# dohlee/metheor

Hardware: AMD Instinct MI355X
Metric: M reads/sec (PDR+LPMD, 150bp WGBS) (higher is better)
Workload: dtype u32; 1 GPU; S-chr19-10M (BASELINE config 2): 10000000 x 150bp reads/GPU, chr19 58.6 Mbp, 2.94 CpG calls/read, fused PDR+LPMD, reference CLI defaults; reads_per_gpu=10000000, cpg_calls_per_gpu=29424182, sites_emitted=726028, parallelism=contig-sharded x1

## Files before the change

metheor_amd/csrc/mth_pdr_lpmd.hip:

```cpp
#include "mth_ctx.h"
#include "mth_tile_dev.h"

#ifndef MTH_TILE_PF
#define MTH_TILE_PF 1
#endif

namespace mth {


constexpr int IDX_GROUPS = 1;
__device__ __forceinline__ void index_safe_hi(const uint32_t *__restrict__ cpg_off, const uint32_t n_reads, const uint32_t n_cpgs,
                                              const uint32_t gtid, DevState *__restrict__ st) {
    uint32_t best = 0;
#pragma unroll
    for (uint32_t k = 0; k < 4; ++k) {
        const uint32_t back = gtid * 4u + k;
        if (back <= n_reads) {
            const uint32_t r = n_reads - back;
            if ((uint64_t)cpg_off[r] + 8u <= (uint64_t)n_cpgs) best = max(best, r);
        }
    }
#pragma unroll
    for (int o = 32; o > 0; o >>= 1) best = max(best, (uint32_t)__shfl_xor((int)best, o, 64));
    if (gtid == 0) st->safe_hi = best;
// ... 218 lines not shown
    if (tid < 4) {
        uint32_t s = 0;
        for (int w = 0; w < B / 64; ++w) s += red[tid][w];
        if (s) atomicAdd(a.bucket + a.nbk + (size_t)(t >> TILE_BUCKET_SHIFT) * 4 + tid, (unsigned long long)s);
    }
}

template <int W, int B, bool WIDE>
__device__ __forceinline__ uint32_t tile_compact(const TileArgs &a, const uint32_t t, const int32_t P0, const uint32_t Wp,
                                                 const uint32_t *cnt, uint32_t *wave_off, const uint32_t out_base) {
    const int tid = threadIdx.x, lane = tid & 63, wave = tid >> 6;
    constexpr int NPOS = WIDE ? W / 2 : W;
    constexpr int PER = NPOS / B;
    static_assert(PER % 4 == 0 && PER <= 32, "uint4 LDS reads, 32-bit mask");
    uint32_t qual = 0;
    if (WIDE) {
#pragma unroll
        for (int q = 0; q < PER / 4; ++q) {
            const uint4 x = reinterpret_cast<const uint4 *>(cnt)[tid * (PER / 4) + q];
            const uint4 y = reinterpret_cast<const uint4 *>(cnt + W / 2)[tid * (PER / 4) + q];
            const uint4 cov = make_uint4(x.x + y.x, x.y + y.y, x.z + y.z, x.w + y.w);
            qual |= (cov.x >= a.min_cov ? 1u : 0u) << (4 * q);
            qual |= (cov.y >= a.min_cov ? 1u : 0u) << (4 * q + 1);
            qual |= (cov.z >= a.min_cov ? 1u : 0u) << (4 * q + 2);
            qual |= (cov.w >= a.min_cov ? 1u : 0u) << (4 * q + 3);
        }
    } else {
        uint32_t below = 0;
#ifdef MTH_TILE_ROT
        static_assert(PER == 16 || WIDE, "the rotation is written for 16 positions per thread");
        const uint32_t rot = ((uint32_t)lane >> 2) & 3u;
#pragma unroll
        for (int q = PER / 4 - 1; q >= 0; --q) {
            const uint4 x = reinterpret_cast<const uint4 *>(cnt)[tid * (PER / 4) + (((uint32_t)q + rot) & 3u)];
            below = __builtin_amdgcn_alignbit(below, (x.w & 0xffffu) - a.min_cov, 31);
            below = __builtin_amdgcn_alignbit(below, (x.z & 0xffffu) - a.min_cov, 31);
            below = __builtin_amdgcn_alignbit(below, (x.y & 0xffffu) - a.min_cov, 31);
            below = __builtin_amdgcn_alignbit(below, (x.x & 0xffffu) - a.min_cov, 31);
        }
        {
            const uint32_t dbl = below | (below << 16);
            below = (dbl >> (16u - 4u * rot)) & 0xffffu;
        }
#else
#pragma unroll
        for (int q = PER / 4 - 1; q >= 0; --q) {
            const uint4 x = reinterpret_cast<const uint4 *>(cnt)[tid * (PER / 4) + q];
            below = __builtin_amdgcn_alignbit(below, (x.w & 0xffffu) - a.min_cov, 31);
            below = __builtin_amdgcn_alignbit(below, (x.z & 0xffffu) - a.min_cov, 31);
            below = __builtin_amdgcn_alignbit(below, (x.y & 0xffffu) - a.min_cov, 31);
            below = __builtin_amdgcn_alignbit(below, (x.x & 0xffffu) - a.min_cov, 31);
        }
#endif
        qual = ~below & (PER == 32 ? 0xffffffffu : (1u << PER) - 1u);
    }
    {
        const int32_t left = (int32_t)Wp - tid * PER;
        qual &= left >= PER ? 0xffffffffu : (left > 0 ? (1u << left) - 1u : 0u);
    }
    const uint32_t mine = __builtin_popcount(qual);
    const uint32_t incl = wave_scan_incl(mine);
    static_assert(B == 256, "four wave totals in one 16-byte LDS word");
    if (lane == 63) wave_off[wave] = incl;
    __syncthreads();
    const uint4 wt = *reinterpret_cast<const uint4 *>(wave_off);
    const uint32_t before = (wave > 0 ? wt.x : 0u) + (wave > 1 ? wt.y : 0u) + (wave > 2 ? wt.z : 0u);
    const uint32_t total = wt.x + wt.y + wt.z + wt.w;
    uint32_t o = out_base + before + incl - mine;
    SiteRec *__restrict__ out = a.scratch + (size_t)t * W;
    while (qual) {
        const uint32_t idx = (uint32_t)tid * PER + (uint32_t)__builtin_ctz(qual);
        qual &= qual - 1;
        SiteRec rr; rr.pos = P0 + (int32_t)idx; rr.pad = 0;
        if (WIDE) { rr.n_conc = cnt[idx]; rr.n_disc = cnt[W / 2 + idx]; }
        else { const uint32_t x = cnt[idx]; rr.n_disc = x >> 16; rr.n_conc = (x & 0xffffu) - rr.n_disc; }
        out[o++] = rr;
    }
    return total;
}

template <typename RelT, int NB>
__device__ __forceinline__ void load_rel(const RelT *__restrict__ rp, int32_t (&r)[NB]) {
    if constexpr (sizeof(RelT) == 1) {
#pragma unroll
        for (int k8 = 0; k8 < NB / 8; ++k8) {
            const u32x2_a1 x = *reinterpret_cast<const u32x2_a1 *>(rp + 8 * k8);
#pragma unroll
            for (int k = 0; k < 4; ++k) { r[8 * k8 + k] = (int32_t)((x.x >> (8 * k)) & 0xffu); r[8 * k8 + 4 + k] = (int32_t)((x.y >> (8 * k)) & 0xffu); }
        }
    } else {
#pragma unroll
        for (int k8 = 0; k8 < NB / 8; ++k8) {
            const u32x4_a2 x = *reinterpret_cast<const u32x4_a2 *>(rp + 8 * k8);
            r[8 * k8] = (int32_t)(x.x & 0xffffu); r[8 * k8 + 1] = (int32_t)(x.x >> 16);
            r[8 * k8 + 2] = (int32_t)(x.y & 0xffffu); r[8 * k8 + 3] = (int32_t)(x.y >> 16);
            r[8 * k8 + 4] = (int32_t)(x.z & 0xffffu); r[8 * k8 + 5] = (int32_t)(x.z >> 16);
            r[8 * k8 + 6] = (int32_t)(x.w & 0xffffu); r[8 * k8 + 7] = (int32_t)(x.w >> 16);
        }
    }
}

#ifdef MTH_TILE_TRACE
#define g_tk4 (*mth_tk4p)
#define g_tk5 (*mth_tk5p)
__device__ unsigned long long mth_tk_dummy[2];
#endif
template <int W, int B, int NB, typename RelT, bool WIDE, bool CLAMP, int MG>
__device__ __forceinline__ uint32_t tile_pass(const TileArgs &a, const uint32_t t, const int32_t T0, const int32_t T1,
                                              const int32_t P0, const uint32_t Wp, const uint32_t lo, const uint32_t hi,
                                              const bool do_lp, const uint32_t out_base, uint32_t *cnt_raw,
                                              uint32_t (*red)[B / 64], uint32_t *wave_off, SlotTabs &tabs
#ifdef MTH_TILE_TRACE
                                              , unsigned long long *mth_tk4p = &mth_tk_dummy[0], unsigned long long *mth_tk5p = &mth_tk_dummy[1]
#endif
                                              ) {
    const int tid = threadIdx.x;
    uint32_t *const cnt = cnt_raw + MG;
    constexpr bool MARGIN = MG > 0 && !WIDE;
    const RelT *__restrict__ rel = reinterpret_cast<const RelT *>(a.cpg_rel);
    constexpr bool PACKED = sizeof(RelT) == 1 && NB == 8;

    uint32_t lp_c = 0, lp_d = 0, n_read = 0, n_valid = 0, bad = 0;
    uint32_t i = lo + tid;
    int32_t s = 0;
    uint32_t o0 = 0, n = 0, mq = 0;
    constexpr bool PF = MTH_TILE_PF && !CLAMP && sizeof(RelT) == 1 && NB == 8;
    uint32_t o1 = 0;
    if (PF) { if (i < hi) { o0 = a.cpg_off[i]; o1 = a.cpg_off[i + 1]; } }
    else if (i < hi) { s = a.read_start[i]; o0 = a.cpg_off[i]; n = a.cpg_off[i + 1] - o0; mq = a.read_mapq[i]; }
    while (i < hi) {
        const uint32_t inext = i + B;
        const bool more = inext < hi;
        uint32_t v[NB];
        int32_t r[NB];
        uint32_t rraw0 = 0, rraw1 = 0;
        uint32_t o0n = 0, o1n = 0;
        if constexpr (PF) {
            n = o1 - o0;
            const uint32_t *__restrict__ cp = a.cpg_pos + o0;
#pragma unroll
            for (int k4 = 0; k4 < NB / 4; ++k4) {
                const u32x4_a4 x = *reinterpret_cast<const u32x4_a4 *>(cp + 4 * k4);
                v[4 * k4] = x.x; v[4 * k4 + 1] = x.y; v[4 * k4 + 2] = x.z; v[4 * k4 + 3] = x.w;
            }
            if (do_lp) { const u32x2_a1 x = *reinterpret_cast<const u32x2_a1 *>(reinterpret_cast<const RelT *>(a.cpg_rel) + o0); rraw0 = x.x; rraw1 = x.y; }
            s = a.read_start[i]; mq = a.read_mapq[i];
            if (more) { o0n = a.cpg_off[inext]; o1n = a.cpg_off[inext + 1]; }
        }
        const bool owned = (s >= T0) && (s < T1);
        const bool lp_ok = do_lp && owned && (mq >= a.lpmd_min_qual);
        if (do_lp && owned) { n_read += 1; n_valid += lp_ok ? 1u : 0u; }
        const bool pdr_ok = a.want_pdr && (n >= a.min_cpgs) && (mq >= a.pdr_min_qual) && (n > 0);
        const bool work = (lp_ok || pdr_ok) && n != 0;
        const int32_t maxd = PACKED ? min(a.max_dist, 255) : min(a.max_dist, 1 << 20);
        const int32_t mind = max(a.min_dist, 0);
        const bool any_lp = maxd >= a.min_dist && maxd >= 0 && __any(work && lp_ok && n > 1);
        if (work) {
            const uint32_t *__restrict__ cp = a.cpg_pos + o0;
            const RelT *__restrict__ rp = rel + o0;
            if (PF) {
                (void)cp; (void)rp;
            } else if (!CLAMP) {
#pragma unroll
                for (int k4 = 0; k4 < NB / 4; ++k4) {
                    const u32x4_a4 x = *reinterpret_cast<const u32x4_a4 *>(cp + 4 * k4);
                    v[4 * k4] = x.x; v[4 * k4 + 1] = x.y; v[4 * k4 + 2] = x.z; v[4 * k4 + 3] = x.w;
                }
                if (any_lp) {
                    if constexpr (PACKED) { const u32x2_a1 x = *reinterpret_cast<const u32x2_a1 *>(rp); rraw0 = x.x; rraw1 = x.y; }
                    else load_rel<RelT, NB>(rp, r);
                }
            } else {
#pragma unroll
                for (int k = 0; k < NB; ++k) v[k] = cp[min((uint32_t)k, n - 1)];
                if (any_lp) {
#pragma unroll
                    for (int k = 0; k < NB; ++k) {
                        const uint32_t rv = (uint32_t)rp[min((uint32_t)k, n - 1)];
                        if constexpr (PACKED) { if (k < 4) rraw0 |= rv << (8 * k); else rraw1 |= rv << (8 * (k - 4)); }
                        else r[k] = (int32_t)rv;
                    }
                }
            }
        const uint32_t sm1 = (uint32_t)(s - 1);
        const uint32_t dead_w = ((MARGIN ? (uint32_t)(P0 - MG + (tid & 63)) : (uint32_t)T0 + (1u << 28)) & 0x7fffffffu) | (v[0] & 0x80000000u);
        const uint32_t n_lp = lp_ok ? min(n, (uint32_t)NB) : 0u;
        uint32_t acc = 0, xmax = (v[0] & 0x7fffffffu) - sm1;
        if constexpr (PACKED) {
            const uint32_t nrow = min(n, 8u);
            const uint4 ma = reinterpret_cast<const uint4 *>(&tabs.mtab[nrow][0])[0], mb = reinterpret_cast<const uint4 *>(&tabs.mtab[nrow][0])[1];
            const uint32_t mk[8] = {ma.x, ma.y, ma.z, ma.w, mb.x, mb.y, mb.z, mb.w};
            uint32_t xs[8];
            xs[0] = xmax;
#pragma unroll
            for (int k = 1; k < 8; ++k) {
                xs[k] = __builtin_amdgcn_bitop3_b32(v[k] - sm1, mk[k], 0x7fffffffu, 0x80);
                v[k] = __builtin_amdgcn_bitop3_b32(v[k], dead_w, mk[k], 0xe4);
                acc = __builtin_amdgcn_bitop3_b32(acc, v[k], v[0], 0xf6);
            }
            xmax = max(max(max(xs[0], xs[1]), max(xs[2], xs[3])), max(max(xs[4], xs[5]), max(xs[6], xs[7])));
        } else {
// ... 51 lines not shown
                    const int32_t dist = rk - (int32_t)rel[o0 + j];
                    if (dist > a.max_dist) break;
                    if (dist < a.min_dist) continue;
                    if ((a.cpg_pos[o0 + j] >> 31) == mk) lp_c += 1; else lp_d += 1;
                }
            }
        }
        if (MARGIN) {
            if (pdr_ok && !bad_it && (uint32_t)s - (uint32_t)(P0 - MG + 1) <= (uint32_t)(W + MG - 1)) {
                const uint32_t one = disc ? 0x10001u : 1u;
                const uint32_t base4 = (uint32_t)(P0 - MG) << 2;
#pragma unroll
                for (int k = 0; k < NB; ++k)
                    atomicAdd(reinterpret_cast<uint32_t *>(reinterpret_cast<char *>(cnt_raw) + ((v[k] << 2) - base4)), one);
                if (any_long) {
                    for (uint32_t k = NB; k < n; ++k) {
                        const uint32_t pk = (a.cpg_pos[o0 + k] & 0x7fffffffu) - (uint32_t)P0;
                        if (pk < Wp) atomicAdd(cnt + pk, one);
                    }
                }
            }
        } else if (!WIDE) {
            const uint32_t one = disc ? 0x10001u : 1u;
            const uint32_t base4 = ((uint32_t)P0 << 2) - (pdr_ok ? 0u : (1u << 30));
            const uint32_t trash4 = (uint32_t)(W + (tid & 63)) << 2;
#pragma unroll
            for (int k = 0; k < NB; ++k) {
                const uint32_t a4 = min((v[k] << 2) - base4, trash4);
                atomicAdd(reinterpret_cast<uint32_t *>(reinterpret_cast<char *>(cnt) + a4), one);
            }
            if (any_long && pdr_ok) {
                for (uint32_t k = NB; k < n; ++k) {
                    const uint32_t pk = (a.cpg_pos[o0 + k] & 0x7fffffffu) - (uint32_t)P0;
                    if (pk < Wp) atomicAdd(cnt + pk, one);
                }
            }
        } else {
            const uint32_t wt = pdr_ok ? Wp : 0u;
            const uint32_t dw = disc ? (uint32_t)(W / 2) : 0u;
            const uint32_t trash = (uint32_t)(W + (tid & 63)) - dw;
#pragma unroll
            for (int k = 0; k < NB; ++k) {
                const uint32_t pk = (v[k] & 0x7fffffffu) - (uint32_t)P0;
                atomicAdd(cnt + ((pk < wt ? pk : trash) + dw), 1u);
            }
            if (any_long && pdr_ok) {
                for (uint32_t k = NB; k < n; ++k) {
                    const uint32_t pk = (a.cpg_pos[o0 + k] & 0x7fffffffu) - (uint32_t)P0;
                    if (pk < Wp) atomicAdd(cnt + dw + pk, 1u);
                }
            }
        }
        }
        if (PF) { o0 = o0n; o1 = o1n; }
        else if (more) { s = a.read_start[inext]; o0 = a.cpg_off[inext]; n = a.cpg_off[inext + 1] - o0; mq = a.read_mapq[inext]; }
        i = inext;
    }
#ifdef MTH_TILE_TRACE
    g_tk4 = __builtin_readcyclecounter();
#endif
    if (bad) atomicOr(const_cast<uint32_t *>(&a.st->err), (uint32_t)ERRB_SPAN);
    if (do_lp) tile_lpmd_partials<B, !WIDE>(a, t, red, lp_c, lp_d, n_read, n_valid);
    __syncthreads();
#ifdef MTH_TILE_TRACE
    g_tk5 = __builtin_readcyclecounter();
#endif
    if (do_lp) tile_lpmd_commit<B>(a, t, red);
    if (!a.want_pdr) return 0u;
    return tile_compact<W, B, WIDE>(a, t, P0, Wp, cnt, wave_off, out_base);
}

#ifndef MTH_TILE_OCC
#define MTH_TILE_OCC 8
#endif
template <int W, int B, int NB, typename RelT, int MG>
__global__ __launch_bounds__(B, MTH_TILE_OCC) void k_pdr_lpmd_tile(const TileArgs a, const uint32_t ntiles) {
    static_assert(MG == 0 || (MG >= 64 && MG % 4 == 0), "the wide passes keep their trash words in the high margin");
    __shared__ __attribute__((aligned(16))) uint32_t cnt[MG ? MG + W + MG : W + 64];
    __shared__ uint32_t red[4][B / 64];
    __shared__ __attribute__((aligned(16))) uint32_t wave_off[B / 64];
    __shared__ __attribute__((aligned(16))) SlotTabs tabs;

    const uint32_t per_xcd = (ntiles + 7) / 8;
    const uint32_t t = (blockIdx.x & 7) * per_xcd + (blockIdx.x >> 3);
    if (t >= ntiles) return;
#ifdef MTH_TILE_TRACE
    unsigned long long tk[8];
    tk[0] = __builtin_readcyclecounter();
#define MTH_TK(k) do { tk[k] = __builtin_readcyclecounter(); } while (0)
#else
#define MTH_TK(k) do {} while (0)
#endif
    const int32_t T0 = a.region_beg + (int32_t)(t * W);
    const int32_t T1 = (int32_t)min((int64_t)T0 + W, (int64_t)a.region_end);

    const uint32_t lo_raw = a.idx2 ? a.idx[t] : a.idx[((uint32_t)T0 - (uint32_t)a.max_span + 1u - (uint32_t)a.idx_base) >> IDX_QSHIFT];
    const uint32_t hi_raw = a.idx2 ? a.idx2[t + 1] : a.idx[(((uint32_t)T0 + (uint32_t)W - (uint32_t)a.idx_base) >> IDX_QSHIFT) + 1];
    const uint32_t safe_hi = a.st->safe_hi;
    auto clear = [&]() {
        for (int i = threadIdx.x; i < W / 4; i += B) reinterpret_cast<uint4 *>(cnt + MG)[i] = make_uint4(0, 0, 0, 0);
    };
    clear();
    slot_tabs_init(tabs, threadIdx.x);
    MTH_TK(1);
    __syncthreads();
    MTH_TK(2);
    const uint32_t lo = min(lo_raw, a.n_reads), hi = min(hi_raw, a.n_reads);
    MTH_TK(3);
    uint32_t rows;
    if (hi - lo <= 65535u) {
        static_assert(NB == 8, "safe_hi is computed for 8 call slots");
        if (hi <= safe_hi)
            rows = tile_pass<W, B, NB, RelT, false, false, MG>(a, t, T0, T1, T0, (uint32_t)(T1 - T0), lo, hi, a.want_lpmd != 0, 0u, cnt, red, wave_off, tabs
#ifdef MTH_TILE_TRACE
                                                               , &tk[4], &tk[5]
#endif
                                                               );
        else
            rows = tile_pass<W, B, NB, RelT, false, true, MG>(a, t, T0, T1, T0, (uint32_t)(T1 - T0), lo, hi, a.want_lpmd != 0, 0u, cnt, red, wave_off, tabs);
    } else {
        const int32_t Tm = (int32_t)min((int64_t)T0 + W / 2, (int64_t)T1);
        rows = tile_pass<W, B, NB, RelT, true, true, MG>(a, t, T0, T1, T0, (uint32_t)(Tm - T0), lo, hi, a.want_lpmd != 0, 0u, cnt, red, wave_off, tabs);
        __syncthreads();
        clear();
        __syncthreads();
        rows += tile_pass<W, B, NB, RelT, true, true, MG>(a, t, T0, T1, Tm, (uint32_t)(T1 - Tm), lo, hi, false, rows, cnt, red, wave_off, tabs);
    }
    if (threadIdx.x == 0) {
        a.tile_cnt[t] = rows;
        if (rows) atomicAdd(a.bucket + (t >> TILE_BUCKET_SHIFT), (unsigned long long)rows);
    }
#ifdef MTH_TILE_TRACE
    MTH_TK(7);
    if (threadIdx.x == 0 && a.trace) { tk[6] = hi - lo; for (int k = 0; k < 8; ++k) a.trace[8 * (size_t)t + k] = tk[k]; }
#endif
}

constexpr uint32_t PT_PASS_ITERS = 255u;

struct RunArgs {
    uint32_t *run_tile0;
    uint32_t *run_rows;
    unsigned long long *run_lpmd;
    DevState *cst;
    uint32_t hint_stride;
    unsigned long long *trace;
};
#ifdef MTH_RUNS_TRACE
#define RT_NOW() __builtin_readcyclecounter()
#define RT_ADD(acc, t0) do { const unsigned long long n__ = RT_NOW(); acc += n__ - t0; t0 = n__; } while (0)
#else
#define RT_NOW() 0ull
#define RT_ADD(acc, t0) do {} while (0)
#endif

__device__ __forceinline__ unsigned long long wave_sum64(uint32_t v) {
// ... 557 lines not shown
        if (wave == 0) mine = lane < nt ? tile_cnt[t0 + lane] : 0u;
        else { const uint32_t u = (bk << TILE_BUCKET_SHIFT) + (tid - 64u); if (u < t0) part = tile_cnt[u]; }
        for (uint32_t b = tid; b < bk; b += 256u) part += (uint32_t)bucket[b];
    }
    const uint32_t incl = wave_scan_incl(mine);
    if (wave == 0) { s_off[lane + 1] = incl; if (lane == 0) s_off[0] = 0u; }
    const uint32_t wsum = wave_sum(part);
    if (lane == 0) s_part[wave] = wsum;
    __syncthreads();
    const uint32_t before = s_part[0] + s_part[1] + s_part[2] + s_part[3];
    const uint32_t total = s_off[nt];
    const uint64_t base = cur + before;
    for (uint32_t r = tid; r < total; r += 256u) {
        uint32_t q = 0;
#pragma unroll
        for (uint32_t step = GATHER2_TILES / 2; step > 0; step >>= 1) q += (s_off[q + step] <= r) ? step : 0u;
        const SiteRec rec = scratch[(size_t)(t0 + q) * tile_w + (r - s_off[q])];
        out_pos[base + r] = rec.pos;
        out_nc[base + r] = rec.n_conc;
        out_nd[base + r] = rec.n_disc;
        out_pdr[base + r] = (float)rec.n_disc / ((float)rec.n_conc + (float)rec.n_disc);
    }
    if (t0 + nt != ntiles) return;
    const uint32_t batch_total = before + total;
    if (tid == 0) {
        const uint32_t nb = reset_first ? 0u : st->n_batches;
        st->n_sites = cur + batch_total;
        batch_cnt[nb] = batch_total;
        st->n_batches = nb + 1;
        if (next_st) next_st->cur_base = cur + batch_total;
        uint32_t e = reset_first ? 0u : st->err;
        if (lane_st) { e |= lane_st->err; lane_st->err = 0; }
        if (lane_st || reset_first) st->err = e;
    }
    if (wave == 0 && (want_lpmd || reset_first)) {
#pragma unroll
        for (int k = 0; k < 4; ++k) {
            unsigned long long x = 0;
            if (want_lpmd) for (uint32_t b = lane; b < nbk; b += 64) x += bucket[nbk + (size_t)b * 4 + k];
#pragma unroll
            for (int o = 32; o > 0; o >>= 1) x += __shfl_down(x, o, 64);
            if (lane == 0) st->lpmd[k] = (reset_first ? 0ll : st->lpmd[k]) + (long long)x;
        }
    }
}

__global__ void k_pipe_seed(const DevState *__restrict__ st, DevState *__restrict__ lane_st) {
    lane_st->cur_base = st->n_sites;
    lane_st->err = 0;
}

constexpr int DENSE_TILE_SHIFT = 12;
constexpr int TILE_MARGIN = 256;
template <int W, int B, typename RelT>
static void launch_tile(const TileArgs &a, uint32_t ntiles, hipStream_t s) {
    const uint32_t grid = ((ntiles + 7) / 8) * 8;
    static const bool no_margin = getenv("MTH_TILE_NO_MARGIN") != nullptr;
    if (a.max_span <= TILE_MARGIN && !no_margin) hipLaunchKernelGGL((k_pdr_lpmd_tile<W, B, 8, RelT, TILE_MARGIN>), dim3(grid), dim3(B), 0, s, a, ntiles);
    else hipLaunchKernelGGL((k_pdr_lpmd_tile<W, B, 8, RelT, 0>), dim3(grid), dim3(B), 0, s, a, ntiles);
}

static uint32_t runs_grid(uint32_t ntiles) {
    static const uint32_t slots = [] {
        int dev = 0, cus = 256;
        if (hipGetDevice(&dev) == hipSuccess) (void)hipDeviceGetAttribute(&cus, hipDeviceAttributeMultiprocessorCount, dev);
        const char *e = getenv("MTH_RUNS_WGS_PER_CU");
        const int per = e && atoi(e) > 0 ? atoi(e) : MTH_RUNS_OCC;
        return (uint32_t)std::max(cus, 1) * (uint32_t)per;
    }();
    return std::max(1u, std::min(slots, ntiles));
}
static void launch_runs(const TileArgs &a, const RunArgs &ra, uint32_t ntiles, uint32_t G, hipStream_t s) {
    static const bool no_margin = getenv("MTH_TILE_NO_MARGIN") != nullptr;
    if (a.max_span <= TILE_MARGIN && !no_margin) hipLaunchKernelGGL((k_pdr_lpmd_runs<(1 << DENSE_TILE_SHIFT), TILE_MARGIN>), dim3(G), dim3(256), 0, s, a, ra, ntiles);
    else hipLaunchKernelGGL((k_pdr_lpmd_runs<(1 << DENSE_TILE_SHIFT), 0>), dim3(G), dim3(256), 0, s, a, ra, ntiles);
}

__global__ __launch_bounds__(256) void k_batch_begin(DevState *__restrict__ lane_st, DevState *__restrict__ cst, const DevState *__restrict__ prep_st,
                                                     unsigned long long *__restrict__ bucket_sums, uint32_t n_bucket_words) {
    if (threadIdx.x == 0) {
        if (cst) cst->cur_base = cst->n_sites;
        lane_st->safe_hi = prep_st->safe_hi;
        if (prep_st->err) atomicOr(&lane_st->err, prep_st->err);
    }
    for (uint32_t w = threadIdx.x; w < n_bucket_words; w += 256) bucket_sums[w] = 0ull;
}
__global__ void k_batch_err(DevState *__restrict__ st, const DevState *__restrict__ prep_st) { if (prep_st->err) atomicOr(&st->err, prep_st->err); }

int build_fine_index(mth_ctx *ctx, const mth_batch_t &b, int32_t idx_base, uint32_t nq, uint32_t *idx, DevState *st) {
    hipStream_t s = ctx->stream;
    LaunchTimer lt(ctx, K_INDEX);
    const uint32_t nb = (b.n_reads / 4 + 1 + BLOCK * IDX_GROUPS - 1) / (BLOCK * IDX_GROUPS);
    hipLaunchKernelGGL(k_build_index<1>, dim3(nb), dim3(BLOCK), 0, s, b.read_start, b.n_reads, idx_base, 0, (int)IDX_QSHIFT, nq,
                       (int)((reinterpret_cast<uintptr_t>(b.read_start) & 15u) == 0), idx, (uint32_t *)nullptr, st,
                       (DevState *)nullptr, (unsigned long long *)nullptr, 0u, b.cpg_off, b.n_cpgs, b.cpg_off, b.n_cpgs ? b.cpg_pos : nullptr);
    MTH_HIP(ctx, hipGetLastError());
    return MTH_OK;
}

int build_read_index(mth_ctx *ctx, const mth_batch_t &b, int tile_w, int32_t &idx_base, uint32_t &ntiles) {
    hipStream_t s = ctx->stream;
    const int64_t region_len = (int64_t)b.region_end - b.region_beg;
    ntiles = (uint32_t)((region_len + tile_w - 1) / tile_w);
    const int32_t ext = ((b.max_span + 2 + IDX_Q - 1) / IDX_Q) * IDX_Q;
    idx_base = b.region_beg - ext;
    const uint32_t nq = (uint32_t)(((int64_t)ntiles * tile_w + ext) >> IDX_QSHIFT) + 2;
    ctx->cur_idx = nullptr;
    if (Prepared *pr = ctx->cur_prep) {
        if (pr->idx_base == idx_base && nq <= pr->nq) {
            ctx->cur_idx = pr->idx.as<uint32_t>();
            hipLaunchKernelGGL(k_batch_err, dim3(1), dim3(1), 0, s, ctx->d_state, (const DevState *)pr->st);
// ... 53 lines not shown
    uint32_t *o_nd = sink ? sink->nd : ctx->out_nd.as<uint32_t>();
    const int64_t region_len = (int64_t)b.region_end - b.region_beg;
    int wide_shift = 0;
    if (b.n_reads && region_len > 0) {
        const double sites_per_bp = (double)b.n_cpgs / (double)b.n_reads / (double)std::max(b.max_span, 1);
        const double reads_per_bp = (double)b.n_reads / (double)region_len;
        double ins_per_read = 0.0;
        if (p.want_pdr) {
            const double lam = (double)b.n_cpgs / (double)b.n_reads;
            const int kmin = (int)std::min<uint32_t>(std::max<uint32_t>(p.pdr_min_cpgs, 1u), 64u) - 1;
            double term = std::exp(-lam), cdf = 0.0;
            for (int k = 0; k < kmin; ++k) { cdf += term; term *= lam / (double)(k + 1); }
            ins_per_read = lam * std::max(0.0, 1.0 - cdf);
        }
        if (sites_per_bp <= 0.012 && reads_per_bp * 4096.0 <= 900.0 && ins_per_read <= 0.6)
        {
            wide_shift = sites_per_bp * 65536.0 <= 0.6 * 1024 && reads_per_bp * 65536.0 <= 4500.0 ? 16 : sites_per_bp * 32768.0 <= 0.6 * 1024 ? 15 : 14;
            while (wide_shift > 14 && (region_len >> wide_shift) < 2 * 7 * 256) --wide_shift;
        }
    }
    if (const char *e = getenv("MTH_PDR_WIDE")) { const int k = atoi(e); wide_shift = k >= 14 && k <= 16 ? k : 0; }
    if (fq && fq->force && wide_shift == 0) wide_shift = 14;
    const int tile_w = wide_shift ? 1 << wide_shift : 4096;
    uint32_t tile_w_rt = 0;
    if (wide_shift) {
        const double slots = 7.0 * 256.0, rounds = (double)region_len / (double)tile_w / slots;
        const double frac = rounds - std::floor(rounds);
        if (rounds > 1.0 && rounds < 8.0 && frac > 0.02 && frac < 0.5) {
            const uint64_t w = (uint64_t)std::ceil((double)region_len / (std::ceil(rounds) * slots));
            const uint32_t wr = (uint32_t)((w + 63) & ~63ull);
            if (wr >= (uint32_t)tile_w / 2 && wr < (uint32_t)tile_w) tile_w_rt = wr;
        }
        if (const char *e = getenv("MTH_PDR_WIDE_W")) { const int k = atoi(e); tile_w_rt = (k >= 1024 && k < tile_w) ? (uint32_t)k & ~63u : 0u; }
    }
    const uint32_t tile_step = tile_w_rt ? tile_w_rt : (uint32_t)tile_w;
    const uint32_t ntiles = (uint32_t)((region_len + tile_step - 1) / tile_step);
    if (ntiles == 0) return MTH_OK;
    const int32_t ext = ((b.max_span + 2 + IDX_Q - 1) / IDX_Q) * IDX_Q;
    const int32_t idx_base = b.region_beg - ext;
    const uint32_t nq = (uint32_t)(((int64_t)ntiles * tile_step + ext) >> IDX_QSHIFT) + 2;

    const char *coarse_env = getenv("MTH_COARSE_INDEX");
    const bool coarse_off = coarse_env && atoi(coarse_env) == 0;
    Prepared *prep = ctx->cur_prep;
    if (prep && !(prep->idx_base == idx_base && nq <= prep->nq)) prep = nullptr;
    const bool coarse = !sink && wide_shift == 0 && !coarse_off && !prep;
    const uint32_t coarse_stride = (ntiles + 2u + 3u) & ~3u;
    if (!prep) MTH_HIP(ctx, b_idx.reserve(coarse ? (size_t)coarse_stride * 2 * 4 : (size_t)(nq + 1) * 4, s));
    const uint32_t *fine_idx = prep ? prep->idx.as<uint32_t>() : nullptr;
    ctx->cur_idx = fine_idx;
    const char *runs_env = getenv("MTH_TILE_RUNS");
    const bool runs = wide_shift == 0 && b.cpg_rel != nullptr && b.n_cpgs < (1u << 30) && runs_env && atoi(runs_env) == 1;
    const uint32_t G = runs ? runs_grid(ntiles) : 0u;
    MTH_HIP(ctx, b_tile_cnt.reserve((size_t)ntiles * 4 * (runs ? 4 : 1), s));
    const uint32_t nbk = (ntiles + (1u << TILE_BUCKET_SHIFT) - 1) >> TILE_BUCKET_SHIFT;
    const uint32_t n_bucket_words = nbk * 5u;
    const size_t run_words = ((size_t)G + 2u) / 2u + ((size_t)G + 1u) / 2u;
    MTH_HIP(ctx, b_bucket.reserve(((size_t)n_bucket_words + run_words + (size_t)G * 4u) * sizeof(unsigned long long), s));
    if (p.want_pdr) MTH_HIP(ctx, b_scratch.reserve((size_t)ntiles * (size_t)tile_w * sizeof(SiteRec), s));

    if (prep) {
        if (runs) hipLaunchKernelGGL(k_batch_err, dim3(1), dim3(1), 0, s, lane_st, (const DevState *)prep->st);
        else hipLaunchKernelGGL(k_batch_begin, dim3(1), dim3(256), 0, s, lane_st, L ? (DevState *)nullptr : cst, (const DevState *)prep->st,
                                b_bucket.as<unsigned long long>(), n_bucket_words);
    } else if (!runs || sink) {
        LaunchTimer lt(ctx, K_INDEX);
        const uint32_t nb = (b.n_reads / 4 + 1 + BLOCK * IDX_GROUPS - 1) / (BLOCK * IDX_GROUPS);
        const int al16 = (int)((reinterpret_cast<uintptr_t>(b.read_start) & 15u) == 0);
        if (coarse)
            hipLaunchKernelGGL(k_build_index<2>, dim3(nb), dim3(BLOCK), 0, s, b.read_start, b.n_reads, b.region_beg - b.max_span + 1, b.region_beg + 1,
                               DENSE_TILE_SHIFT, ntiles + 1u, al16, b_idx.as<uint32_t>(), b_idx.as<uint32_t>() + coarse_stride, lane_st,
                               L ? (DevState *)nullptr : cst, b_bucket.as<unsigned long long>(), n_bucket_words, b.cpg_off, b.n_cpgs, b.cpg_off,
                               b.n_cpgs ? b.cpg_pos : nullptr);
        else
            hipLaunchKernelGGL(k_build_index<1>, dim3(nb), dim3(BLOCK), 0, s, b.read_start, b.n_reads, idx_base, 0, (int)IDX_QSHIFT, nq, al16,
                               b_idx.as<uint32_t>(), (uint32_t *)nullptr, lane_st, L ? (DevState *)nullptr : cst,
                               b_bucket.as<unsigned long long>(), n_bucket_words, b.cpg_off, b.n_cpgs, b.cpg_off, b.n_cpgs ? b.cpg_pos : nullptr);
    } else if (b.n_reads && b.n_cpgs) {
        hipLaunchKernelGGL(k_minus_one_check, dim3(std::min<uint32_t>((b.n_reads + 255) / 256, 64u)), dim3(256), 0, s, b.read_start, b.cpg_off, b.cpg_pos,
                           b.n_reads, b.n_cpgs, lane_st);
    }
    TileArgs a;
    a.read_start = b.read_start; a.read_mapq = b.read_mapq; a.cpg_off = b.cpg_off; a.cpg_pos = b.cpg_pos;
    a.cpg_rel = b.cpg_rel ? (const void *)b.cpg_rel : (const void *)b.cpg_rel16;
    a.idx = fine_idx ? fine_idx : b_idx.as<uint32_t>(); a.idx2 = coarse ? b_idx.as<uint32_t>() + coarse_stride : nullptr; a.st = lane_st;
    a.tile_cnt = b_tile_cnt.as<uint32_t>(); a.bucket = b_bucket.as<unsigned long long>(); a.nbk = nbk;
    a.scratch = b_scratch.as<SiteRec>();
    a.region_beg = b.region_beg; a.region_end = b.region_end; a.idx_base = idx_base; a.max_span = b.max_span;
    a.n_reads = b.n_reads; a.n_cpgs = b.n_cpgs;
    a.min_cov = p.pdr_min_depth > 1 ? p.pdr_min_depth : 1;
    a.min_cpgs = p.pdr_min_cpgs;
    a.min_dist = p.lpmd_min_distance; a.max_dist = p.lpmd_max_distance;
    a.pdr_min_qual = p.pdr_min_qual; a.lpmd_min_qual = p.lpmd_min_qual;
    a.want_pdr = p.want_pdr; a.want_lpmd = p.want_lpmd;
    a.tile_w_rt = tile_w_rt;
    RunArgs ra;
    ra.run_tile0 = reinterpret_cast<uint32_t *>(b_bucket.as<unsigned long long>() + n_bucket_words);
    ra.run_rows = ra.run_tile0 + (((size_t)G + 2u) / 2u) * 2u;
    ra.run_lpmd = b_bucket.as<unsigned long long>() + n_bucket_words + run_words;
    ra.cst = L ? (DevState *)nullptr : cst;
    ra.trace = nullptr;
#ifdef MTH_RUNS_TRACE
    static unsigned long long *d_rtrace = nullptr;
    if (!d_rtrace) (void)hipMalloc((void **)&d_rtrace, 8 * 8 * 4 * 4096);
    ra.trace = G <= 4096 ? d_rtrace : nullptr;
#endif
    ra.hint_stride = (uint32_t)std::max(1.0, std::ceil((double)b.n_reads / (double)ntiles * (1.0 + (double)b.max_span / (double)tile_w) * 1.3 / 63.0));
#ifdef MTH_TILE_TRACE
    static unsigned long long *d_ttrace = nullptr;
    if (!d_ttrace) (void)hipMalloc((void **)&d_ttrace, 8 * 8 * 262144);
    a.trace = ntiles <= 262144 ? d_ttrace : nullptr;
#endif
    {
        LaunchTimer lt(ctx, wide_shift ? K_WIDE : K_TILE);
        const bool r8 = b.cpg_rel != nullptr;
        if (wide_shift && fq && ntiles <= fq->max_tiles) { launch_tile_fused(a, *fq, ntiles, wide_shift, r8, s); fq->taken = true; fq->ntiles = ntiles; }
        else if (wide_shift) launch_tile_wide(a, ntiles, wide_shift, r8, s);
        else if (runs) launch_runs(a, ra, ntiles, G, s);
        else if (r8) launch_tile<(1 << DENSE_TILE_SHIFT), 256, uint8_t>(a, ntiles, s); else launch_tile<(1 << DENSE_TILE_SHIFT), 256, uint16_t>(a, ntiles, s);
    }
    {
        LaunchTimer lt(ctx, K_GATHER);
        int reset_first = 0;
        if (L) {
            if (ctx->pipe_tail >= 0 && ctx->pipe_tail != li) MTH_HIP(ctx, hipStreamWaitEvent(s, ctx->lane[ctx->pipe_tail].done, 0));
            reset_first = ctx->reset_pending ? 1 : 0;
            ctx->reset_pending = false;
        }
        static const bool gather1 = getenv("MTH_GATHER") && atoi(getenv("MTH_GATHER")) == 1;
        if (runs)
            hipLaunchKernelGGL(k_gather_runs, dim3(p.want_pdr ? G : 1u), dim3(256), 0, s, b_scratch.as<SiteRec>(),
                               b_tile_cnt.as<uint32_t>(), ra.run_tile0, ra.run_rows, ra.run_lpmd, G,
                               p.want_pdr ? 0 : 1, (int)p.want_lpmd, cst, L ? (const DevState *)L->st : (const DevState *)cst,
                               L ? ctx->lane[li ^ 1].st : (DevState *)nullptr, L ? L->st : (DevState *)nullptr, reset_first,
                               bcnt, (uint32_t)tile_w / 4u, o_pos, o_pdr, o_nc, o_nd);
        else if (gather1)
            hipLaunchKernelGGL(k_gather, dim3(p.want_pdr ? (ntiles + GATHER_WAVES - 1) / GATHER_WAVES : 1u), dim3(p.want_pdr ? 64 * GATHER_WAVES : 64), 0, s, b_scratch.as<SiteRec>(),
                               b_tile_cnt.as<uint32_t>(), b_bucket.as<unsigned long long>(), nbk, ntiles,
                               p.want_pdr ? 0 : 1, (int)p.want_lpmd, cst, L ? (const DevState *)L->st : (const DevState *)cst,
                               L ? ctx->lane[li ^ 1].st : (DevState *)nullptr, L ? L->st : (DevState *)nullptr, reset_first,
                               bcnt, (uint32_t)tile_w, o_pos, o_pdr, o_nc, o_nd);
        else
            hipLaunchKernelGGL(k_gather2, dim3(p.want_pdr ? (ntiles + GATHER2_TILES - 1) / GATHER2_TILES : 1u), dim3(256), 0, s, b_scratch.as<SiteRec>(),
                               b_tile_cnt.as<uint32_t>(), b_bucket.as<unsigned long long>(), nbk, ntiles,
                               p.want_pdr ? 0 : 1, (int)p.want_lpmd, cst, L ? (const DevState *)L->st : (const DevState *)cst,
                               L ? ctx->lane[li ^ 1].st : (DevState *)nullptr, L ? L->st : (DevState *)nullptr, reset_first,
                               bcnt, (uint32_t)tile_w, o_pos, o_pdr, o_nc, o_nd);
        if (L) { MTH_HIP(ctx, hipEventRecord(L->done, s)); ctx->pipe_tail = li; }
    }
#ifdef MTH_RUNS_TRACE
    if (getenv("MTH_RUNS_TRACE_OUT") && runs && G <= 4096) {
        (void)hipStreamSynchronize(s);
        std::vector<unsigned long long> tt(8 * 4 * (size_t)G);
        (void)hipMemcpy(tt.data(), d_rtrace, tt.size() * 8, hipMemcpyDeviceToHost);
        FILE *f = fopen(getenv("MTH_RUNS_TRACE_OUT"), "wb");
        if (f) { fwrite(tt.data(), 8, tt.size(), f); fclose(f); }
    }
#endif
#ifdef MTH_TILE_TRACE
    if (getenv("MTH_TILE_TRACE_OUT") && ntiles <= 262144) {
        (void)hipStreamSynchronize(s);
        std::vector<unsigned long long> tt(8 * (size_t)ntiles);
        (void)hipMemcpy(tt.data(), d_ttrace, tt.size() * 8, hipMemcpyDeviceToHost);
        FILE *f = fopen(getenv("MTH_TILE_TRACE_OUT"), "wb");
        if (f) { fwrite(tt.data(), 8, tt.size(), f); fclose(f); }
    }
#endif
    MTH_HIP(ctx, hipGetLastError());
    return MTH_OK;
}

// ... 2 lines not shown
```

metheor_amd/csrc/mth_tile_dev.h:

```cpp
#pragma once
#include "mth_common.h"
#include "mth_lpmd_bytes.h"

namespace mth {

#define MTH_DPP(v, ctrl, rmask, bctl) ((uint32_t)__builtin_amdgcn_update_dpp(0, (int)(v), (ctrl), (rmask), 0xf, (bctl)))
__device__ __forceinline__ uint32_t wave_sum(uint32_t v) {
    v += MTH_DPP(v, 0xb1 , 0xf, true);
    v += MTH_DPP(v, 0x4e , 0xf, true);
    v += MTH_DPP(v, 0x141 , 0xf, true);
    v += MTH_DPP(v, 0x140 , 0xf, true);
    return __builtin_amdgcn_readlane(v, 0) + __builtin_amdgcn_readlane(v, 16) + __builtin_amdgcn_readlane(v, 32) +
           __builtin_amdgcn_readlane(v, 48);
}
__device__ __forceinline__ uint32_t wave_scan_incl(uint32_t v) {
    v += MTH_DPP(v, 0x111 , 0xf, true);
    v += MTH_DPP(v, 0x112 , 0xf, true);
    v += MTH_DPP(v, 0x114 , 0xf, true);
    v += MTH_DPP(v, 0x118 , 0xf, true);
    v += MTH_DPP(v, 0x142 , 0xa, false);
    v += MTH_DPP(v, 0x143 , 0xc, false);
    return v;
}

// ... 1 lines not shown

struct TileArgs {
    const int32_t  *read_start;
    const uint8_t  *read_mapq;
    const uint32_t *cpg_off;
    const uint32_t *cpg_pos;
    const void     *cpg_rel;
    const uint32_t *idx;
    const uint32_t *idx2;
    const DevState *st;
    uint32_t *tile_cnt;
    unsigned long long *bucket;
    uint32_t nbk;
    SiteRec  *scratch;
    int32_t region_beg, region_end, idx_base, max_span;
    uint32_t n_reads, n_cpgs;
    uint32_t min_cov;
    uint32_t min_cpgs;
    int32_t  min_dist, max_dist;
    uint8_t  pdr_min_qual, lpmd_min_qual, want_pdr, want_lpmd;
    uint32_t tile_w_rt;
#ifdef MTH_TILE_TRACE
    unsigned long long *trace;
#endif
};

typedef uint32_t u32x4_a4 __attribute__((ext_vector_type(4), aligned(4)));
typedef uint32_t u32x2_a1 __attribute__((ext_vector_type(2), aligned(1)));
typedef uint32_t u32x4_a2 __attribute__((ext_vector_type(4), aligned(2)));

void launch_tile_wide(const TileArgs &a, uint32_t ntiles, int shift, bool rel8, hipStream_t s);

struct FusedQuartet {
    uint8_t force;
    uint8_t force_heavy;
    uint8_t min_qual;
    unsigned long long *qs;
    unsigned long long row_cap;
    uint32_t max_tiles;
    uint32_t *tile_flag;
    unsigned long long *tile_row0;
    uint32_t *tile_rows;
    int32_t *out_pos; uint32_t *out_cnt; float *out_me, *out_pm; uint32_t *out_depth;
    bool taken;
    uint32_t ntiles;
};
void launch_tile_fused(const TileArgs &a, const FusedQuartet &q, uint32_t ntiles, int shift, bool rel8, hipStream_t s);

struct SlotTabs {
    uint32_t mtab[9][8];
    uint32_t dtab[9][8];
    LpMask   m8[9][8];
};
__device__ __forceinline__ void slot_tabs_init(SlotTabs &T, const int tid) {
    if (tid < 144) (&T.m8[0][0].w0)[tid] = lpmd_bytes_mask((uint32_t)tid >> 4, ((uint32_t)tid >> 1) & 7u, (uint32_t)tid & 1u);
    if (tid < 72) {
        const uint32_t nn = (uint32_t)tid >> 3, c = (uint32_t)tid & 7u;
        T.mtab[nn][c] = c < nn ? 0xffffffffu : 0u;
        auto dead = [&](uint32_t k) { return k >= 8u ? 0x2400u : (k >= nn ? 0x400u * (k + 1u) : 0u); };
        const uint32_t lo = c < 4 ? 2u * c : 2u * (c - 4u) + 1u;
        T.dtab[nn][c] = dead(lo) | (dead(lo + 1u) << 16);
    }
}
__device__ __forceinline__ uint32_t bfi(uint32_t mask, uint32_t a, uint32_t b) { return (a & mask) | (b & ~mask); }

__device__ __forceinline__ void lpmd_pairs_fields16(const uint32_t (&v)[8], const uint32_t rraw0, const uint32_t rraw1, const uint32_t *drow,
                                                    const uint32_t mind, const uint32_t maxd, uint32_t &lp_c, uint32_t &lp_d) {
    uint32_t SQ[4], SO[4], Q[4], O[4];
#pragma unroll
    for (int e = 0; e < 4; ++e) SQ[e] = __builtin_amdgcn_perm(v[2 * e + 1], v[2 * e], 0x070c030cu);
#pragma unroll
    for (int e = 0; e < 3; ++e) SO[e] = __builtin_amdgcn_perm(v[2 * e + 2], v[2 * e + 1], 0x070c030cu);
    SO[3] = __builtin_amdgcn_perm(0u, v[7], 0x070c030cu);
    Q[0] = __builtin_amdgcn_perm(0u, rraw0, 0x0c010c00u); Q[1] = __builtin_amdgcn_perm(0u, rraw0, 0x0c030c02u);
    Q[2] = __builtin_amdgcn_perm(0u, rraw1, 0x0c010c00u); Q[3] = __builtin_amdgcn_perm(0u, rraw1, 0x0c030c02u);
    O[0] = __builtin_amdgcn_perm(0u, rraw0, 0x0c020c01u); O[1] = __builtin_amdgcn_perm(rraw1, rraw0, 0x0c040c03u);
    O[2] = __builtin_amdgcn_perm(0u, rraw1, 0x0c020c01u); O[3] = __builtin_amdgcn_perm(0u, rraw1, 0x0c0c0c03u);
    {
        const uint4 da = reinterpret_cast<const uint4 *>(drow)[0], db = reinterpret_cast<const uint4 *>(drow)[1];
        Q[0] += da.x; Q[1] += da.y; Q[2] += da.z; Q[3] += da.w; O[0] += db.x; O[1] += db.y; O[2] += db.z; O[3] += db.w;
    }
    const uint32_t KA = (0x8000u - mind) * 0x10001u, KB = (0x8000u + maxd) * 0x10001u;
    uint32_t accIN = 0, accDD = 0;
#pragma unroll
    for (int g = 1; g < 8; ++g) {
        uint32_t orB = 0;
#pragma unroll
        for (int m = 0; m < 4; ++m) {
            const int li = (g & 1) ? (g - 1) / 2 + m : g / 2 + m;
            if (li > 3) break;
            const uint32_t later = (g & 1) ? O[li] : Q[li], sl = (g & 1) ? SO[li] : SQ[li];
            const uint32_t D = later - Q[m];
            const uint32_t Bw = KB - D;
            const uint32_t IN = __builtin_amdgcn_bitop3_b32(D + KA, Bw, 0x80008000u, 0x80);
            const uint32_t DD = IN & (sl ^ SQ[m]);
            accIN += __builtin_popcount(IN);
            accDD += __builtin_popcount(DD);
            orB |= Bw;
        }
        if (!__any((orB & 0x80008000u) != 0u)) break;
    }
    lp_c += accIN - accDD;
    lp_d += accDD;
}

__device__ __forceinline__ void lpmd_pairs8(const uint32_t (&v)[8], const uint32_t rraw0, const uint32_t rraw1, const uint32_t n_lp,
                                            const SlotTabs &T, const int32_t mind, const int32_t maxd, uint32_t &lp_c, uint32_t &lp_d) {
    if (lpmd_bytes_domain(mind, maxd))
        lpmd_pairs_bytes(rraw0, rraw1, lpmd_state_bytes(v[0], v[1], v[2], v[3]), lpmd_state_bytes(v[4], v[5], v[6], v[7]), &T.m8[n_lp][0],
// ... 8 lines not shown
```

Measured before the change: 123,000 M reads/s.

## Add 128-thread tile kernel with two-stream software-pipelined read loads

Adds a 128-thread block variant of the dense tile kernel and makes it the default on the LPMD path. In that variant each thread keeps two reads in flight and interleaves them, so the position, rel, start and mapq loads for one read are issued before the other read is processed, hiding global load latency. It also lowers launch bounds occupancy to 5 and skips the margin variant for B=128. The trade is higher register pressure and lower occupancy, plus extra loads clamped to the last read at the tail.

```diff
diff --git a/metheor_amd/csrc/mth_pdr_lpmd.hip b/metheor_amd/csrc/mth_pdr_lpmd.hip
--- a/metheor_amd/csrc/mth_pdr_lpmd.hip
+++ b/metheor_amd/csrc/mth_pdr_lpmd.hip
@@ -294,7 +294,7 @@
             below = __builtin_amdgcn_alignbit(below, (x.x & 0xffffu) - a.min_cov, 31);
         }
 #endif
-        qual = ~below & (PER == 32 ? 0xffffffffu : (1u << PER) - 1u);
+        qual = ~below & (uint32_t)((1ull << PER) - 1ull);
     }
     {
         const int32_t left = (int32_t)Wp - tid * PER;
@@ -302,12 +302,19 @@
     }
     const uint32_t mine = __builtin_popcount(qual);
     const uint32_t incl = wave_scan_incl(mine);
-    static_assert(B == 256, "four wave totals in one 16-byte LDS word");
+    static_assert(B == 256 || B == 128, "the B / 64 wave totals in one 16- or 8-byte LDS word");
     if (lane == 63) wave_off[wave] = incl;
     __syncthreads();
-    const uint4 wt = *reinterpret_cast<const uint4 *>(wave_off);
-    const uint32_t before = (wave > 0 ? wt.x : 0u) + (wave > 1 ? wt.y : 0u) + (wave > 2 ? wt.z : 0u);
-    const uint32_t total = wt.x + wt.y + wt.z + wt.w;
+    uint32_t before, total;
+    if constexpr (B == 256) {
+        const uint4 wt = *reinterpret_cast<const uint4 *>(wave_off);
+        before = (wave > 0 ? wt.x : 0u) + (wave > 1 ? wt.y : 0u) + (wave > 2 ? wt.z : 0u);
+        total = wt.x + wt.y + wt.z + wt.w;
+    } else {
+        const uint2 wt = *reinterpret_cast<const uint2 *>(wave_off);
+        before = wave > 0 ? wt.x : 0u;
+        total = wt.x + wt.y;
+    }
     uint32_t o = out_base + before + incl - mine;
     SiteRec *__restrict__ out = a.scratch + (size_t)t * W;
     while (qual) {
@@ -363,32 +370,20 @@
     constexpr bool PACKED = sizeof(RelT) == 1 && NB == 8;
 
     uint32_t lp_c = 0, lp_d = 0, n_read = 0, n_valid = 0, bad = 0;
-    uint32_t i = lo + tid;
-    int32_t s = 0;
-    uint32_t o0 = 0, n = 0, mq = 0;
     constexpr bool PF = MTH_TILE_PF && !CLAMP && sizeof(RelT) == 1 && NB == 8;
-    uint32_t o1 = 0;
-    if (PF) { if (i < hi) { o0 = a.cpg_off[i]; o1 = a.cpg_off[i + 1]; } }
-    else if (i < hi) { s = a.read_start[i]; o0 = a.cpg_off[i]; n = a.cpg_off[i + 1] - o0; mq = a.read_mapq[i]; }
-    while (i < hi) {
-        const uint32_t inext = i + B;
-        const bool more = inext < hi;
-        uint32_t v[NB];
+    constexpr bool TWO = PF && B == 128;
+    auto request = [&](const uint32_t i, const uint32_t o0, uint32_t (&v)[NB], uint32_t &rraw0, uint32_t &rraw1, int32_t &s, uint32_t &mq) __attribute__((always_inline)) {
+        const uint32_t *__restrict__ cp = a.cpg_pos + o0;
+#pragma unroll
+        for (int k4 = 0; k4 < NB / 4; ++k4) {
+            const u32x4_a4 x = *reinterpret_cast<const u32x4_a4 *>(cp + 4 * k4);
+            v[4 * k4] = x.x; v[4 * k4 + 1] = x.y; v[4 * k4 + 2] = x.z; v[4 * k4 + 3] = x.w;
+        }
+        if (do_lp || TWO) { const u32x2_a1 x = *reinterpret_cast<const u32x2_a1 *>(reinterpret_cast<const RelT *>(a.cpg_rel) + o0); rraw0 = x.x; rraw1 = x.y; }
+        s = a.read_start[i]; mq = a.read_mapq[i];
+    };
+    auto chunk = [&](const int32_t s, const uint32_t mq, const uint32_t o0, const uint32_t n, uint32_t (&v)[NB], uint32_t rraw0, uint32_t rraw1) __attribute__((always_inline)) {
         int32_t r[NB];
-        uint32_t rraw0 = 0, rraw1 = 0;
-        uint32_t o0n = 0, o1n = 0;
-        if constexpr (PF) {
-            n = o1 - o0;
-            const uint32_t *__restrict__ cp = a.cpg_pos + o0;
-#pragma unroll
-            for (int k4 = 0; k4 < NB / 4; ++k4) {
-                const u32x4_a4 x = *reinterpret_cast<const u32x4_a4 *>(cp + 4 * k4);
-                v[4 * k4] = x.x; v[4 * k4 + 1] = x.y; v[4 * k4 + 2] = x.z; v[4 * k4 + 3] = x.w;
-            }
-            if (do_lp) { const u32x2_a1 x = *reinterpret_cast<const u32x2_a1 *>(reinterpret_cast<const RelT *>(a.cpg_rel) + o0); rraw0 = x.x; rraw1 = x.y; }
-            s = a.read_start[i]; mq = a.read_mapq[i];
-            if (more) { o0n = a.cpg_off[inext]; o1n = a.cpg_off[inext + 1]; }
-        }
         const bool owned = (s >= T0) && (s < T1);
         const bool lp_ok = do_lp && owned && (mq >= a.lpmd_min_qual);
         if (do_lp && owned) { n_read += 1; n_valid += lp_ok ? 1u : 0u; }
@@ -546,9 +541,49 @@
             }
         }
         }
-        if (PF) { o0 = o0n; o1 = o1n; }
-        else if (more) { s = a.read_start[inext]; o0 = a.cpg_off[inext]; n = a.cpg_off[inext + 1] - o0; mq = a.read_mapq[inext]; }
-        i = inext;
+    };
+    if constexpr (TWO) {
+        uint32_t ia = lo + tid, ib = ia + B;
+        if (ia < hi) {
+            const uint32_t last = hi - 1u;
+            uint32_t oa0, oa1, ob0, ob1, va[NB], vb[NB], ra0, ra1, rb0, rb1, mqa, mqb;
+            int32_t sa, sb;
+            { const uint32_t jb = min(ib, last); oa0 = a.cpg_off[ia]; oa1 = a.cpg_off[ia + 1]; ob0 = a.cpg_off[jb]; ob1 = a.cpg_off[jb + 1]; }
+            request(ia, oa0, va, ra0, ra1, sa, mqa);
+            while (ia < hi) {
+                const uint32_t ian = ia + 2 * B, ibn = ib + 2 * B;
+                const uint32_t ja = min(ian, last), jb = min(ibn, last);
+                const uint32_t oa0n = a.cpg_off[ja], oa1n = a.cpg_off[ja + 1];
+                request(min(ib, last), ob0, vb, rb0, rb1, sb, mqb);
+                chunk(sa, mqa, oa0, oa1 - oa0, va, ra0, ra1);
+                const uint32_t ob0n = a.cpg_off[jb], ob1n = a.cpg_off[jb + 1];
+                request(ja, oa0n, va, ra0, ra1, sa, mqa);
+                if (ib < hi) chunk(sb, mqb, ob0, ob1 - ob0, vb, rb0, rb1);
+                ia = ian; ib = ibn; oa0 = oa0n; oa1 = oa1n; ob0 = ob0n; ob1 = ob1n;
+            }
+        }
+    } else {
+        uint32_t i = lo + tid;
+        int32_t s = 0;
+        uint32_t o0 = 0, o1 = 0, n = 0, mq = 0;
+        if (PF) { if (i < hi) { o0 = a.cpg_off[i]; o1 = a.cpg_off[i + 1]; } }
+        else if (i < hi) { s = a.read_start[i]; o0 = a.cpg_off[i]; n = a.cpg_off[i + 1] - o0; mq = a.read_mapq[i]; }
+        while (i < hi) {
+            const uint32_t inext = i + B;
+            const bool more = inext < hi;
+            uint32_t v[NB];
+            uint32_t rraw0 = 0, rraw1 = 0;
+            uint32_t o0n = 0, o1n = 0;
+            if constexpr (PF) {
+                n = o1 - o0;
+                request(i, o0, v, rraw0, rraw1, s, mq);
+                if (more) { o0n = a.cpg_off[inext]; o1n = a.cpg_off[inext + 1]; }
+            }
+            chunk(s, mq, o0, n, v, rraw0, rraw1);
+            if (PF) { o0 = o0n; o1 = o1n; }
+            else if (more) { s = a.read_start[inext]; o0 = a.cpg_off[inext]; n = a.cpg_off[inext + 1] - o0; mq = a.read_mapq[inext]; }
+            i = inext;
+        }
     }
 #ifdef MTH_TILE_TRACE
     g_tk4 = __builtin_readcyclecounter();
@@ -568,7 +603,7 @@
 #define MTH_TILE_OCC 8
 #endif
 template <int W, int B, int NB, typename RelT, int MG>
-__global__ __launch_bounds__(B, MTH_TILE_OCC) void k_pdr_lpmd_tile(const TileArgs a, const uint32_t ntiles) {
+__global__ __launch_bounds__(B, B == 128 ? 5 : MTH_TILE_OCC) void k_pdr_lpmd_tile(const TileArgs a, const uint32_t ntiles) {
     static_assert(MG == 0 || (MG >= 64 && MG % 4 == 0), "the wide passes keep their trash words in the high margin");
     __shared__ __attribute__((aligned(16))) uint32_t cnt[MG ? MG + W + MG : W + 64];
     __shared__ uint32_t red[4][B / 64];
@@ -595,7 +630,7 @@
         for (int i = threadIdx.x; i < W / 4; i += B) reinterpret_cast<uint4 *>(cnt + MG)[i] = make_uint4(0, 0, 0, 0);
     };
     clear();
-    slot_tabs_init(tabs, threadIdx.x);
+    slot_tabs_init<B>(tabs, threadIdx.x);
     MTH_TK(1);
     __syncthreads();
     MTH_TK(2);
@@ -1259,11 +1294,14 @@
 
 constexpr int DENSE_TILE_SHIFT = 12;
 constexpr int TILE_MARGIN = 256;
+#ifndef MTH_TILE_B_DEFAULT
+#define MTH_TILE_B_DEFAULT 128
+#endif
 template <int W, int B, typename RelT>
 static void launch_tile(const TileArgs &a, uint32_t ntiles, hipStream_t s) {
     const uint32_t grid = ((ntiles + 7) / 8) * 8;
     static const bool no_margin = getenv("MTH_TILE_NO_MARGIN") != nullptr;
-    if (a.max_span <= TILE_MARGIN && !no_margin) hipLaunchKernelGGL((k_pdr_lpmd_tile<W, B, 8, RelT, TILE_MARGIN>), dim3(grid), dim3(B), 0, s, a, ntiles);
+    if (B == 256 && a.max_span <= TILE_MARGIN && !no_margin) hipLaunchKernelGGL((k_pdr_lpmd_tile<W, 256, 8, RelT, TILE_MARGIN>), dim3(grid), dim3(256), 0, s, a, ntiles);
     else hipLaunchKernelGGL((k_pdr_lpmd_tile<W, B, 8, RelT, 0>), dim3(grid), dim3(B), 0, s, a, ntiles);
 }
 
@@ -1423,6 +1461,8 @@
     const char *runs_env = getenv("MTH_TILE_RUNS");
     const bool runs = wide_shift == 0 && b.cpg_rel != nullptr && b.n_cpgs < (1u << 30) && runs_env && atoi(runs_env) == 1;
     const uint32_t G = runs ? runs_grid(ntiles) : 0u;
+    int tile_b = L ? MTH_TILE_B_DEFAULT : 256;
+    if (const char *e = getenv("MTH_TILE_B")) { const int k = atoi(e); if (k == 128 || k == 256) tile_b = k; }
     MTH_HIP(ctx, b_tile_cnt.reserve((size_t)ntiles * 4 * (runs ? 4 : 1), s));
     const uint32_t nbk = (ntiles + (1u << TILE_BUCKET_SHIFT) - 1) >> TILE_BUCKET_SHIFT;
     const uint32_t n_bucket_words = nbk * 5u;
@@ -1488,6 +1528,7 @@
         if (wide_shift && fq && ntiles <= fq->max_tiles) { launch_tile_fused(a, *fq, ntiles, wide_shift, r8, s); fq->taken = true; fq->ntiles = ntiles; }
         else if (wide_shift) launch_tile_wide(a, ntiles, wide_shift, r8, s);
         else if (runs) launch_runs(a, ra, ntiles, G, s);
+        else if (r8 && tile_b == 128) launch_tile<(1 << DENSE_TILE_SHIFT), 128, uint8_t>(a, ntiles, s);
         else if (r8) launch_tile<(1 << DENSE_TILE_SHIFT), 256, uint8_t>(a, ntiles, s); else launch_tile<(1 << DENSE_TILE_SHIFT), 256, uint16_t>(a, ntiles, s);
     }
     {
diff --git a/metheor_amd/csrc/mth_tile_dev.h b/metheor_amd/csrc/mth_tile_dev.h
--- a/metheor_amd/csrc/mth_tile_dev.h
+++ b/metheor_amd/csrc/mth_tile_dev.h
@@ -77,9 +77,10 @@
     uint32_t dtab[9][8];
     LpMask   m8[9][8];
 };
-__device__ __forceinline__ void slot_tabs_init(SlotTabs &T, const int tid) {
-    if (tid < 144) (&T.m8[0][0].w0)[tid] = lpmd_bytes_mask((uint32_t)tid >> 4, ((uint32_t)tid >> 1) & 7u, (uint32_t)tid & 1u);
-    if (tid < 72) {
+template <int B = 256>
+__device__ __forceinline__ void slot_tabs_init(SlotTabs &T, const int tid0) {
+    for (int tid = tid0; tid < 144; tid += B) (&T.m8[0][0].w0)[tid] = lpmd_bytes_mask((uint32_t)tid >> 4, ((uint32_t)tid >> 1) & 7u, (uint32_t)tid & 1u);
+    for (int tid = tid0; tid < 72; tid += B) {
         const uint32_t nn = (uint32_t)tid >> 3, c = (uint32_t)tid & 7u;
         T.mtab[nn][c] = c < nn ? 0xffffffffu : 0u;
         auto dead = [&](uint32_t k) { return k >= 8u ? 0x2400u : (k >= nn ? 0x400u * (k + 1u) : 0u); };
```

Result: faster. 129,700 M reads/s, median of 6 (+5.4%).
